# Yasas1994/Jaeger

Hardware: AMD Instinct MI355X
Metric: Mbp/s classified (1500bp frags) (higher is better)
Workload: dtype f16x3 (split-f16, f32 accumulate)

## Files before the change

jaeger_amd/csrc/jg_conv_f16_impl.h:

```cpp
#include <stdio.h>
#include <stdlib.h>
#include <type_traits>

#include "jg_common.h"

#include "jg_conv_dev.h"

namespace {


#ifdef JG_STAMP
static __device__ unsigned long long jg_stamp_acc[8];
#define JG_ST_DECL unsigned long long st_[8] = {0, 0, 0, 0, 0, 0, 0, 0}; unsigned long long st_t = __builtin_amdgcn_s_memtime(); const unsigned long long st_t0 = st_t
#define JG_ST(idx) do { const unsigned long long n_ = __builtin_amdgcn_s_memtime(); st_[idx] += n_ - st_t; st_t = n_; } while (0)
#define JG_ST_END do { st_[5] = __builtin_amdgcn_s_memtime() - st_t0; if (lane == 0) { for (int q_ = 0; q_ < 8; ++q_) atomicAdd(&jg_stamp_acc[q_], st_[q_]); } } while (0)
#else
#define JG_ST_DECL
#define JG_ST(idx)
#define JG_ST_END
#endif

#ifndef JG_PRIO
#define JG_PRIO 1
#endif
// ... 6 lines not shown
#ifndef JG_PAIRED
#define JG_PAIRED 1
#endif
#define JG_PRIO_MAIN() do { if (JG_PRIO) __builtin_amdgcn_s_setprio(2); } while (0)
#define JG_PRIO_EPI() do { if (JG_PRIO) __builtin_amdgcn_s_setprio(0); } while (0)

template <int K, unsigned EP, bool LUT = false, bool FLAT = false, int CW = 128, bool TANH = false, bool PIPE = false>
__global__ __launch_bounds__(LUT ? JG_LUT_WAVES * 64 : HT) __attribute__((amdgpu_waves_per_eu(K == 5 ? 2 : 1, 2)))
void conv_f16x3_kernel(ConvHArgs a) {
  constexpr int NTHR = LUT ? JG_LUT_WAVES * 64 : HT;
  constexpr int WA = K - 2;
  constexpr bool NARROW = !LUT && (CW == 64 || CW == 32);
  constexpr bool GEN = CW != 128;
  const int ch0 = GEN ? a.ch0 : 0;
  const int L_res = GEN ? a.L_res : a.L_out;
  constexpr int TM = NARROW ? 2 : 4;
  constexpr int TN = (NARROW && CW == 32) ? 1 : 2;
  constexpr int STRIPS = HM / (TM * 32);
  extern __shared__ __attribute__((aligned(16))) uint4 lds[];
  const int tid = threadIdx.x, lane = tid & 63;
  const int wid = __builtin_amdgcn_readfirstlane(tid >> 6);
  const int wm = LUT ? (wid & 1) : (NARROW ? wid : (wid >> 1));
  const int wn = LUT ? ((GEN && a.lut_one_half) ? 0 : (int)(blockIdx.x & 1u)) : (NARROW ? 0 : (wid & 1));
  const int i = lane & 31, h = lane >> 5;
  const int lut_sh = (LUT && !(GEN && a.lut_one_half)) ? 1 : 0;
  const int vgrid = (int)(gridDim.x >> lut_sh);
  int vb = (int)(blockIdx.x >> lut_sh);
  if ((vgrid & 7) == 0) vb = (vb & 7) * (vgrid >> 3) + (vb >> 3);
  constexpr int TPER = LUT ? JG_LUT_WAVES / 2 : NT;
  const int tsub = LUT ? (wid >> 1) : 0;
  const int rows_a = HM + (K - 1) * a.dil;
  const int a_items = NT * 4 * rows_a;
  uint4 *Abuf = lds;
  uint4 *Wbuf = lds + 2 * a_items;
  const int lut_rows = a.k * (a.lut_vocab + 1);
  float *epiL = LUT ? reinterpret_cast<float *>(lds) + lut_rows * LUT_RS
                    : reinterpret_cast<float *>(Wbuf + K * W_ITEMS);
  for (int q = tid; q < a.n_epi_rows * 2 * HN; q += NTHR) epiL[q] = a.epi[q];
  const unsigned lds0 = (unsigned)(size_t)(__attribute__((address_space(3))) void *)lds;
  const unsigned ldsA = __builtin_amdgcn_readfirstlane(lds0 + wid * 1024);
  const unsigned ldsW = __builtin_amdgcn_readfirstlane(lds0 + 2 * a_items * 16 + wid * 1024);

  const int n_tiles = FLAT ? a.flat_tiles : a.rows * a.tiles_m;
  const int n_pairs = (n_tiles + TPER - 1) / TPER;
  auto resolve = [&](const Tile &tile, int local, int len, int &row, int &p) -> bool {
    if constexpr (!FLAT) {
      row = tile.rowblk;
      p = tile.m0 + local;
      return tile.valid && p >= 0 && p < len;
    }
    const int v = tile.T * HM + local;
    if (v < 0 || !tile.valid) { row = 0; p = 0; return false; }
    int g, u, f;
    udivmod24(v, a.flat_wp, a.flat_inv_wp, g, u);
    udivmod24(u, a.flat_p, a.flat_inv_p, f, p);
    row = g * a.flat_frames + f;
    return f < a.flat_frames && p < len && row < a.rows;
  };
  int my_pairs = 0;
  if (vb < n_pairs) my_pairs = (n_pairs - 1 - vb) / vgrid + 1;
  if (my_pairs == 0) return;

  unsigned a_pk[A_ITERS];
#pragma unroll
  for (int it = 0; it < A_ITERS; ++it) {
    const int q = tid + it * HT;
    const int ph = q / rows_a;
    a_pk[it] = ((unsigned)(ph >> 2) << 20) | ((unsigned)(ph & 3) << 16) | (unsigned)(q - ph * rows_a);
  }
  unsigned w_voff[W_ITERS];
#pragma unroll
  for (int it = 0; it < W_ITERS; ++it) {
    const int q = tid + it * HT;
    w_voff[it] = (unsigned)((((q >> 8) * K * a.cc_in * 2 + ((q >> 7) & 1)) * HN + (q & (HN - 1))) * 16);
  }

  auto tiles_of = [&](int pass, Tile *t) {
#pragma unroll
    for (int u = 0; u < NT; ++u) {
      const int T = (vb + pass * vgrid) * TPER + tsub + u;
      const int Tc = min(T, n_tiles - 1);
      t[u].rowblk = Tc / a.tiles_m;
      t[u].m0 = (Tc - t[u].rowblk * a.tiles_m) * HM;
      t[u].valid = T < n_tiles;
      t[u].T = Tc;
    }
  };

  const uint8_t *bsrc = a.ids != nullptr ? a.ids : a.mask_in;
  unsigned char raw[A_ITERS];
  unsigned x_voff[A_ITERS];
  unsigned x_ok = 0;
  auto piece_pos = [&](const Tile *tl2, int it, int &pc, bool &inr) -> int {
    const int a_u = (int)(a_pk[it] >> 20), a_r = (int)(a_pk[it] & 0xffff);
    int rb, p;
    inr = resolve(tl2[0], a_r - a.pad_left, a.L_in, rb, p) && a_u < NT;
    pc = min(max(p, 0), a.L_in - 1);
    if constexpr (FLAT) rb = min(rb, a.rows - 1);
    return rb;
  };
  auto load_bytes = [&](const Tile *tl2) {
    if (bsrc != nullptr) {
#pragma unroll
      for (int it = 0; it < A_ITERS; ++it) {
        int pc; bool inr;
        const int rb = piece_pos(tl2, it, pc, inr);
        raw[it] = bsrc[(size_t)rb * a.L_in + pc];
      }
    } else {
#pragma unroll
      for (int it = 0; it < A_ITERS; ++it) raw[it] = 1;
    }
  };
  auto build_pieces = [&](const Tile *tl2) {
    x_ok = 0;
#pragma unroll
    for (int it = 0; it < A_ITERS; ++it) {
      int pc; bool inr;
      const int rb = piece_pos(tl2, it, pc, inr);
      const unsigned ph = (a_pk[it] >> 16) & 3;
      const unsigned byte = raw[it];
      bool keep;
      if (a.ids != nullptr) {
        x_voff[it] = (byte * a.cc_in * 4 + ph) * 16;
        keep = byte != 0 || !a.mask_from_ids;
      } else {
        x_voff[it] = (unsigned)(((rb * a.cc_row * 4 + (int)ph) * a.L_in + pc) * 16);
        keep = byte != 0;
      }
      if (inr && keep) x_ok |= 1u << it;
    }
  };
  const char *x_base = a.ids != nullptr ? reinterpret_cast<const char *>(a.embh)
                                        : reinterpret_cast<const char *>(a.xh);
  const unsigned x_cc_stride = a.ids != nullptr ? 4u * 16u : 4u * (unsigned)a.L_in * 16u;

  const bool x_last_wave = __builtin_amdgcn_readfirstlane((int)((A_ITERS - 1) * HT + wid * 64 < 4 * rows_a)) != 0;
  auto issue_w = [&](int cc, int t) {
    if (a.dbg & 16) return;
    const char *sb = reinterpret_cast<const char *>(a.wh) + ((size_t)(t * a.cc_in * 2 + cc * 2) * HN) * 16;
#pragma unroll
    for (int it = 0; it < W_ITERS; ++it) glds16(sb, w_voff[it], ldsW + t * (W_ITEMS * 16) + it * (HT * 16));
  };
  auto issue_x = [&](int cc, int buf) {
    if (a.dbg & 8) return;
    const char *sb = x_base + (size_t)cc * x_cc_stride;
    const unsigned dst = ldsA + buf * (a_items * 16);
#pragma unroll
    for (int it = 0; it < A_ITERS - 1; ++it) glds16_nt(sb, x_voff[it], dst + it * (HT * 16));
    if (x_last_wave) {
      if ((a_pk[A_ITERS - 1] >> 20) < NT) glds16_nt(sb, x_voff[A_ITERS - 1], dst + (A_ITERS - 1) * (HT * 16));
    }
  };
  auto zero_fill = [&](int buf) {
    uint4 *A = Abuf + buf * a_items;
#pragma unroll
    for (int it = 0; it < A_ITERS; ++it)
      if ((a_pk[it] >> 20) < NT && !((x_ok >> it) & 1u)) A[tid + it * HT] = make_uint4(0u, 0u, 0u, 0u);
  };

  f32x16 acc[TM][TN];
  auto zero_acc = [&]() {
#pragma unroll
    for (int tm = 0; tm < TM; ++tm)
#pragma unroll
      for (int tn = 0; tn < TN; ++tn)
#pragma unroll
        for (int r = 0; r < 16; ++r) acc[tm][tn][r] = 0.f;
  };
  zero_acc();

  const int w_frag = h * HN + wn * 64 + i;
  const int x_frag = h * rows_a + wm * (TM * 32) + i;

  Tile cur[NT], np[NT];
  JG_ST_DECL;
  tiles_of(0, cur);
  tiles_of(1, np);
  unsigned char *stage = reinterpret_cast<unsigned char *>(epiL + JG_EPI_ROWS * 2 * HN) + wid * 256;
  unsigned char nxt[4] = {0, 0, 0, 0};
  auto lut_fetch = [&](const Tile &tl) {
#pragma unroll
    for (int q4 = 0; q4 < 4; ++q4) {
      const int p = tl.m0 + wm * (TM * 32) - a.pad_left + lane + 64 * q4;
      const int pc = min(max(p, 0), a.L_in - 1);
      const unsigned char b = a.ids[(size_t)tl.rowblk * a.L_in + pc];
      nxt[q4] = (tl.valid && p >= 0 && p < a.L_in) ? b : (unsigned char)a.lut_vocab;
    }
  };
  if constexpr (LUT) {
    float4 *T4 = reinterpret_cast<float4 *>(lds);
    const float4 *src = reinterpret_cast<const float4 *>(a.lut) + (size_t)wn * lut_rows * 16;
    for (int q = tid; q < lut_rows * 16; q += NTHR) T4[(q >> 4) * (LUT_RS / 4) + (q & 15)] = src[q];
    lut_fetch(cur[0]);
    __syncthreads();
  } else {
    load_bytes(cur);
    build_pieces(cur);
    load_bytes(np);
    issue_x(0, 0);
#pragma unroll
    for (int t = 0; t < ((K == 5 && JG_PAIRED) ? 4 : WA); ++t) issue_w(0, t);
  }
  int xc = 0;
#ifdef JG_VALU_PROBE
  float probe[8];
#pragma unroll
  for (int q = 0; q < 8; ++q) probe[q] = (float)(lane + q);
#endif
  JG_PRIO_MAIN();
  for (int pass = 0; pass < my_pairs; ++pass) {
    if constexpr (LUT) {
#pragma unroll
      for (int q4 = 0; q4 < 4; ++q4) stage[lane + 64 * q4] = nxt[q4];
      lut_fetch(np[0]);
      __builtin_amdgcn_s_waitcnt(0xc07f);
      __builtin_amdgcn_wave_barrier();
      const float *Tl = reinterpret_cast<const float *>(lds) + 4 * h;
      for (int t = 0; t < a.k; ++t) {
#pragma unroll
        for (int tm = 0; tm < TM; ++tm) {
          const int rowi = stage[tm * 32 + i + t * a.dil];
          const float *r = Tl + (t * (a.lut_vocab + 1) + rowi) * LUT_RS;
#pragma unroll
          for (int tn = 0; tn < TN; ++tn)
#pragma unroll
            for (int g = 0; g < 4; ++g) {
              const float4 v = *reinterpret_cast<const float4 *>(r + tn * 32 + 8 * g);
              acc[tm][tn][4 * g + 0] += v.x; acc[tm][tn][4 * g + 1] += v.y;
              acc[tm][tn][4 * g + 2] += v.z; acc[tm][tn][4 * g + 3] += v.w;
            }
        }
      }
      __builtin_amdgcn_wave_barrier();
    }
    if constexpr (PIPE) {
      static_assert(K == 5 && !LUT && CW == 128, "the pipelined main loop is built for the 128-channel five-tap convs");
      constexpr int DIL = 3;
      struct XF { uint4 h[2], l[2]; };
      struct WF { uint4 h[2], l[2]; };
      XF xf[2];
      WF wf[2];
      const uint4 *Wb = Wbuf + w_frag;
      auto ldx = [&](XF &f, const uint4 *A, int t, int tp) {
#pragma unroll
        for (int tq = 0; tq < 2; ++tq) {
          f.h[tq] = A[(tp * 2 + tq) * 32 + t * DIL];
          f.l[tq] = A[2 * rows_a + (tp * 2 + tq) * 32 + t * DIL];
        }
      };
      auto ldw = [&](WF &f, int t) {
#pragma unroll
        for (int tn = 0; tn < 2; ++tn) {
          f.h[tn] = Wb[t * W_ITEMS + tn * 32];
          f.l[tn] = Wb[t * W_ITEMS + 2 * HN + tn * 32];
        }
      };
      auto mm = [&](auto zero_c, const WF &w, const XF &x, int tp, auto &&between) {
        constexpr bool ZERO = decltype(zero_c)::value;
#pragma unroll
        for (int tq = 0; tq < 2; ++tq)
#pragma unroll
          for (int tn = 0; tn < 2; ++tn) {
            f32x16 &c = acc[tp * 2 + tq][tn];
            const half8 wh = *reinterpret_cast<const half8 *>(&w.h[tn]), wl = *reinterpret_cast<const half8 *>(&w.l[tn]);
            const half8 xh = *reinterpret_cast<const half8 *>(&x.h[tq]), xl = *reinterpret_cast<const half8 *>(&x.l[tq]);
            if constexpr (ZERO) {
              const f32x16 z = {0.f, 0.f, 0.f, 0.f, 0.f, 0.f, 0.f, 0.f, 0.f, 0.f, 0.f, 0.f, 0.f, 0.f, 0.f, 0.f};
              c = __builtin_amdgcn_mfma_f32_32x32x16_f16(wh, xl, z, 0, 0, 0);
            } else {
              c = __builtin_amdgcn_mfma_f32_32x32x16_f16(wh, xl, c, 0, 0, 0);
            }
            c = __builtin_amdgcn_mfma_f32_32x32x16_f16(wl, xh, c, 0, 0, 0);
            c = __builtin_amdgcn_mfma_f32_32x32x16_f16(wh, xh, c, 0, 0, 0);
            between(tq * 2 + tn);
          }
      };
      const bool last_pass_ = pass == my_pairs - 1;
      wait_vm<2 * W_ITERS>();
      zero_fill(0);
      __syncthreads();
      ldw(wf[0], 0);
      ldx(xf[0], Abuf + x_frag, 0, 0);
      for (int cp = 0; cp < a.cc_in / 2; ++cp) {
#pragma unroll
        for (int half = 0; half < 2; ++half) {
          const int cc = 2 * cp + half;
          const bool last_chunk = cc == a.cc_in - 1;
          const bool tail = last_chunk && last_pass_;
          const int ncc = last_chunk ? 0 : cc + 1;
          const uint4 *A = Abuf + half * a_items + x_frag;
          const uint4 *An = Abuf + (half ^ 1) * a_items + x_frag;
#pragma unroll
          for (int g = 0; g < 10; ++g) {
            const int t = g >> 1, tp = g & 1;
            const bool step_end = g == 3 || g == 7 || g == 9;
            const bool pass_end = g == 9 && last_chunk;
            if (step_end && !pass_end) {
              if (g == 3) {
                if (tail) wait_vm<W_ITERS>();
                else if (x_last_wave) wait_vm<W_ITERS + A_ITERS>();
                else wait_vm<W_ITERS + A_ITERS - 1>();
              } else if (g == 7) {
                if (tail) wait_vm<0>();
                else if (x_last_wave) wait_vm<2 * W_ITERS + A_ITERS>();
                else wait_vm<2 * W_ITERS + A_ITERS - 1>();
              } else {
                wait_vm<2 * W_ITERS>();
                zero_fill(half ^ 1);
              }
              __syncthreads();
// ... 334 lines not shown
#pragma unroll
          for (int r = 0; r < 16; ++r) pool_acc[r] = -INFINITY;
        }
        if (!(a.dbg & 32)) {
#pragma unroll
          for (int j = 0; j < 2; ++j) {
            f32x2 v[4];
#pragma unroll
            for (int r = 0; r < 4; ++r) v[r] = f32x2{x[8 * j + 2 * r], x[8 * j + 2 * r + 1]};
            auto st_affine = [&](int row) {
              const float *pr = epiL + (row * 2) * HN + nb + 4 * h + 16 * j;
              const float4 sc0 = *reinterpret_cast<const float4 *>(pr), sc1 = *reinterpret_cast<const float4 *>(pr + 8);
              const float4 of0 = *reinterpret_cast<const float4 *>(pr + HN), of1 = *reinterpret_cast<const float4 *>(pr + HN + 8);
              v[0] = __builtin_elementwise_fma(v[0], f32x2{sc0.x, sc0.y}, f32x2{of0.x, of0.y});
              v[1] = __builtin_elementwise_fma(v[1], f32x2{sc0.z, sc0.w}, f32x2{of0.z, of0.w});
              v[2] = __builtin_elementwise_fma(v[2], f32x2{sc1.x, sc1.y}, f32x2{of1.x, of1.y});
              v[3] = __builtin_elementwise_fma(v[3], f32x2{sc1.z, sc1.w}, f32x2{of1.z, of1.w});
            };
            auto st_add = [&]() {
              const u32x4 qh = j == 0 ? q.sh0 : q.sh1, ql = j == 0 ? q.sl0 : q.sl1;
              unsigned hx = qh[0], hy = qh[1], hz = qh[2], hw_ = qh[3];
              unsigned lx = ql[0], ly = ql[1], lz = ql[2], lw_ = ql[3];
              swap32(hx, hz); swap32(hy, hw_);
              swap32(lx, lz); swap32(ly, lw_);
              v[0] += f32x2{mix_sum<0>(hx, lx), mix_sum<1>(hx, lx)};
              v[1] += f32x2{mix_sum<0>(hy, ly), mix_sum<1>(hy, ly)};
              v[2] += f32x2{mix_sum<0>(hz, lz), mix_sum<1>(hz, lz)};
              v[3] += f32x2{mix_sum<0>(hw_, lw_), mix_sum<1>(hw_, lw_)};
            };
            auto st_gelu = [&]() {
#pragma unroll
              for (int r = 0; r < 4; ++r) v[r] = fast_gelu2(v[r]);
            };
            auto st_nmd = [&]() {
              const f32x2 mk2 = {mk, mk};
#pragma unroll
              for (int r = 0; r < 4; ++r) nmd2[4 * j + r] = __builtin_elementwise_fma(v[r], mk2, nmd2[4 * j + r]);
            };
            st_affine(0);
            if constexpr (EP & JG_EP_NMD1) st_nmd();
            if constexpr (N1 == 1) st_affine(1);
            if constexpr (HAS_ADD) st_add();
            if constexpr (EP & JG_EP_ACT1) st_gelu();
            if constexpr (EP & JG_EP_NMD2) st_nmd();
            if constexpr (N2 == 1) st_affine(N1 ? 2 : 1);
            if constexpr (EP & JG_EP_ACT2) st_gelu();
            if (a.out_f16s) {
              unsigned hp[4], lp[4];
#pragma unroll
              for (int r = 0; r < 4; ++r) {
                typedef _Float16 half2_t __attribute__((ext_vector_type(2)));
                const half2_t hh = {(_Float16)v[r].x, (_Float16)v[r].y};
                hp[r] = *reinterpret_cast<const unsigned *>(&hh);
                const half2_t ll = {(_Float16)mix_rem<0>(v[r].x, hp[r]), (_Float16)mix_rem<1>(v[r].y, hp[r])};
                lp[r] = *reinterpret_cast<const unsigned *>(&ll);
              }
              vmax = fmaxf(fmaxf(vmax, fmaxf(fabsf(v[0].x), fabsf(v[0].y))), fmaxf(fabsf(v[1].x), fabsf(v[1].y)));
              vmax = fmaxf(fmaxf(vmax, fmaxf(fabsf(v[2].x), fabsf(v[2].y))), fmaxf(fabsf(v[3].x), fabsf(v[3].y)));
              vnan = vnan || __builtin_isunordered(v[0].x, v[0].y) || __builtin_isunordered(v[1].x, v[1].y) ||
                     __builtin_isunordered(v[2].x, v[2].y) || __builtin_isunordered(v[3].x, v[3].y);
              swap32(hp[0], hp[2]); swap32(hp[1], hp[3]);
              swap32(lp[0], lp[2]); swap32(lp[1], lp[3]);
              if (live && !(a.dbg & 64)) {
                uint4 *yh = reinterpret_cast<uint4 *>(a.y);
                const unsigned it4 = ob[tm] + (unsigned)(2 * tn + j) * L4;
                const u32x4 vhi = {hp[0], hp[1], hp[2], hp[3]}, vlo = {lp[0], lp[1], lp[2], lp[3]};
                st_stream(vhi, reinterpret_cast<u32x4 *>(yh + it4));
                st_stream(vlo, reinterpret_cast<u32x4 *>(yh + it4 + 2u * (unsigned)a.L_out));
              }
            } else if (a.pool_out != nullptr) {
#pragma unroll
              for (int r = 0; r < 4; ++r) {
                pool_acc[8 * j + 2 * r] = mk != 0.f ? fmaxf(pool_acc[8 * j + 2 * r], v[r].x) : pool_acc[8 * j + 2 * r];
                pool_acc[8 * j + 2 * r + 1] = mk != 0.f ? fmaxf(pool_acc[8 * j + 2 * r + 1], v[r].y) : pool_acc[8 * j + 2 * r + 1];
              }
            } else if (live && !(a.dbg & 64)) {
              float *yf = reinterpret_cast<float *>(a.y) + (size_t)om[tm] * a.cout + nb + 4 * h + 16 * j;
              *reinterpret_cast<float4 *>(yf) = make_float4(v[0].x, v[0].y, v[1].x, v[1].y);
              *reinterpret_cast<float4 *>(yf + 8) = make_float4(v[2].x, v[2].y, v[3].x, v[3].y);
            }
          }
        }
        if (b + 2 < 8) fetch(q, b + 2);
        if (tm == 3) {
          if constexpr (HAS_NMD) {
            float na[16];
#pragma unroll
            for (int r = 0; r < 8; ++r) { na[2 * r] = nmd2[r].x; na[2 * r + 1] = nmd2[r].y; }
            const float rv = lane_reduce(na, [](float x_, float y_) { return x_ + y_; });
            int ch;
            const size_t slot = reduced_slot(tn, ch);
            if (i < 16 && tile.valid) a.nmd_out[slot] = rv;
          }
          if (a.pool_out != nullptr) {
            const float rv = lane_reduce(pool_acc, [](float x_, float y_) { return fmaxf(x_, y_); });
            int ch;
            const size_t slot = reduced_slot(tn, ch);
            if (i < 16 && tile.valid) a.pool_out[slot] = rv;
          }
        }
      };
#pragma unroll
      for (int bp = 0; bp < 4; ++bp) {
        do_block(2 * bp, in0);
        do_block(2 * bp + 1, in1);
      }
      if ((!(vmax <= 65000.0f) || vnan) && a.overflow != nullptr && a.dbg == 0) atomicOr(a.overflow, 1);
      JG_PRIO_MAIN();
    } else {
      JG_PRIO_EPI();
      float vmax = 0.f;
      bool vnan = false;
      float nmd_acc[16];
      float nmd_acc2[16];
      struct Pre {
        uint2 sh[4], sl[4];
        unsigned char mkb;
      };
      auto swap32 = [](unsigned &lo_half_keeps, unsigned &hi_half_keeps) {
        const auto r = __builtin_amdgcn_permlane32_swap(lo_half_keeps, hi_half_keeps, false, false);
        lo_half_keeps = r[0];
        hi_half_keeps = r[1];
      };
      auto item4 = [&](int row, int mc, int nb, int j) -> unsigned {
        const int G = ((nb + ch0) >> 3) + 2 * j + h;
        return (unsigned)(((row * (a.cout_pad >> 4) + (G >> 1)) * 4 + (G & 1)) * a.L_out + mc);
      };
      const bool psplit = GEN && a.psplit != 0;
      const int L_st = psplit ? ((a.L_out + 1) >> 1) : a.L_out;
      auto item4_out = [&](int row, int mc, int nb, int j) -> unsigned {
        if constexpr (GEN) {
          if (psplit) {
            const int G = ((nb + ch0) >> 3) + 2 * j + h, CC = a.cout_pad >> 4;
            return (unsigned)(((row * 2 * CC + (mc & 1) * CC + (G >> 1)) * 4 + (G & 1)) * L_st + (mc >> 1));
          }
        }
        return item4(row, mc, nb, j);
      };
      auto out_pos = [&](const Tile &tile, int tm, int &row, int &mc) -> bool {
        int p;
        bool live = resolve(tile, (wm * TM + tm) * 32 + i, L_res, row, p);
        if constexpr (GEN) {
          if (a.ostride == 2) {
            live = live && !(p & 1);
            p >>= 1;
          }
        }
        mc = live ? p : 0;
        if constexpr (FLAT) {
          if (!live) row = min(max(row, 0), a.rows - 1);
        }
        return live;
      };
      auto prefetch = [&](Pre &p, const Tile &tile, int tm, int tn) {
        const int nb = (wn * 2 + tn) * 32;
        int orow, mc;
        out_pos(tile, tm, orow, mc);
        p.mkb = a.mask_out != nullptr ? a.mask_out[(size_t)orow * a.L_out + mc] : (unsigned char)1;
        if (a.addh != nullptr && !(a.dbg & 128)) {
#pragma unroll
          for (int j = 0; j < 2; ++j) {
            const unsigned it4 = item4(orow, mc, (!GEN || nb + ch0 + 16 * j < a.cout) ? nb : 0, j);
            typedef unsigned u32x4 __attribute__((ext_vector_type(4)));
            const u32x4 nh = ld_stream(reinterpret_cast<const u32x4 *>(a.addh + it4));
            const u32x4 nl = ld_stream(reinterpret_cast<const u32x4 *>(a.addh + it4 + 2u * (unsigned)a.L_out));
            uint4 vh = make_uint4(nh[0], nh[1], nh[2], nh[3]);
            uint4 vl = make_uint4(nl[0], nl[1], nl[2], nl[3]);
            swap32(vh.x, vh.z); swap32(vh.y, vh.w);
            swap32(vl.x, vl.z); swap32(vl.y, vl.w);
            p.sh[2 * j] = make_uint2(vh.x, vh.y);  p.sh[2 * j + 1] = make_uint2(vh.z, vh.w);
            p.sl[2 * j] = make_uint2(vl.x, vl.y);  p.sl[2 * j + 1] = make_uint2(vl.z, vl.w);
          }
        } else {
#pragma unroll
          for (int g = 0; g < 4; ++g) p.sh[g] = p.sl[g] = make_uint2(0u, 0u);
        }
      };
      auto epi_block = [&](f32x16 &x, const Tile &tile, int tm, int tn) {
        Pre p;
        prefetch(p, tile, tm, tn);
        const int nb = (wn * 2 + tn) * 32;
        int orow_, mc_;
        const bool live = out_pos(tile, tm, orow_, mc_);
        const float mk = p.mkb != 0 ? 1.f : 0.f;
        auto st_affine = [&](int row) {
          const float *pr = epiL + (row * 2) * HN + nb + 4 * h;
#pragma unroll
          for (int g = 0; g < 4; ++g) {
            const float4 sc = *reinterpret_cast<const float4 *>(pr + 8 * g);
            const float4 of = *reinterpret_cast<const float4 *>(pr + HN + 8 * g);
            x[4 * g + 0] = fmaf(x[4 * g + 0], sc.x, of.x);
            x[4 * g + 1] = fmaf(x[4 * g + 1], sc.y, of.y);
            x[4 * g + 2] = fmaf(x[4 * g + 2], sc.z, of.z);
            x[4 * g + 3] = fmaf(x[4 * g + 3], sc.w, of.w);
          }
        };
        auto st_dyt = [&](int row, float alpha, int use_mask) {
          const float *pr = epiL + (row * 2) * HN + nb + 4 * h;
          const float mm = use_mask ? mk : 1.0f;
#pragma unroll
          for (int g = 0; g < 4; ++g) {
            const float4 ga = *reinterpret_cast<const float4 *>(pr + 8 * g);
            const float4 be = *reinterpret_cast<const float4 *>(pr + HN + 8 * g);
            x[4 * g + 0] = (fast_tanh(alpha * x[4 * g + 0]) * ga.x + be.x) * mm;
            x[4 * g + 1] = (fast_tanh(alpha * x[4 * g + 1]) * ga.y + be.y) * mm;
            x[4 * g + 2] = (fast_tanh(alpha * x[4 * g + 2]) * ga.z + be.z) * mm;
            x[4 * g + 3] = (fast_tanh(alpha * x[4 * g + 3]) * ga.w + be.w) * mm;
          }
        };
        auto st_add = [&]() {
#pragma unroll
          for (int g = 0; g < 4; ++g) {
            x[4 * g + 0] += mix_sum<0>(p.sh[g].x, p.sl[g].x);
            x[4 * g + 1] += mix_sum<1>(p.sh[g].x, p.sl[g].x);
            x[4 * g + 2] += mix_sum<0>(p.sh[g].y, p.sl[g].y);
            x[4 * g + 3] += mix_sum<1>(p.sh[g].y, p.sl[g].y);
          }
        };
        auto st_gelu = [&]() {
          constexpr bool TANH_ONLY = TANH || EP == JG_EP_RUNTIME ||
                                     (EP != JG_EP_GENERIC && ((((EP >> 1) & 3) == 2) || (((EP >> 6) & 3) == 2)));
          if (TANH_ONLY || a.act_kind == JG_ACT_GELU_TANH) {
#pragma unroll
            for (int r = 0; r < 16; ++r) x[r] = fast_gelu(x[r]);
          } else if (a.act_kind == JG_ACT_GELU_ERF) {
#pragma unroll
            for (int r = 0; r < 16; ++r) x[r] = gelu_erf(x[r]);
          } else {
#pragma unroll
            for (int r = 0; r < 16; ++r) x[r] = fmaxf(x[r], 0.0f);
          }
        };
        auto st_nmd = [&](int which = 0) {
          const float mkl = live ? mk : 0.f;
          if constexpr (EP == JG_EP_RUNTIME) {
            if (which) {
#pragma unroll
              for (int r = 0; r < 16; ++r) nmd_acc2[r] = fmaf(x[r], mkl, nmd_acc2[r]);
              return;
            }
          }
#pragma unroll
          for (int r = 0; r < 16; ++r) nmd_acc[r] = fmaf(x[r], mkl, nmd_acc[r]);
        };
        if constexpr (EP == JG_EP_GENERIC) {
          for (int q = 0; q < ((a.dbg & 32) ? 0 : a.n_hst); ++q) {
            const HStageArg st = a.hst[q];
            switch (st.kind) {
              case JG_HST_AFFINE: st_affine(st.pad_); break;
              case JG_HST_DYT: st_dyt(st.pad_, st.f0, st.arg); break;
              case JG_HST_ADD: st_add(); break;
              case JG_HST_ACT:
#pragma unroll
                for (int r = 0; r < 16; ++r) x[r] = jg_act(x[r], st.arg);
                break;
              case JG_HST_NMD: st_nmd(); break;
              case JG_HST_MASKMUL:
#pragma unroll
                for (int r = 0; r < 16; ++r) x[r] *= mk;
                break;
              default: break;
            }
          }
        } else if constexpr (EP == JG_EP_RUNTIME) {
          const unsigned e_ = a.ep_rt;
          const int n1 = (int)((e_ >> 1) & 3u), n2 = (int)((e_ >> 6) & 3u);
          st_affine(0);
          if (e_ & JG_EP_NMD1) st_nmd(0);
          if (n1 == 1) st_affine(1);
          else if (n1 == 2) st_dyt(1, a.alpha1, a.dytmask1);
          if (e_ & JG_EP_ADD) st_add();
          if (e_ & JG_EP_ACT1) st_gelu();
          if (e_ & JG_EP_NMD2) st_nmd((e_ & JG_EP_NMD1) ? 1 : 0);
          if (n2 == 1) st_affine(n1 ? 2 : 1);
          else if (n2 == 2) st_dyt(n1 ? 2 : 1, a.alpha2, a.dytmask2);
          if (e_ & JG_EP_ACT2) st_gelu();
        } else if (!(a.dbg & 32)) {
          constexpr int N1 = (EP >> 1) & 3, N2 = (EP >> 6) & 3;
          st_affine(0);
          if constexpr (EP & JG_EP_NMD1) st_nmd();
          if constexpr (N1 == 1) st_affine(1);
          if constexpr (N1 == 2) st_dyt(1, a.alpha1, a.dytmask1);
          if constexpr (EP & JG_EP_ADD) st_add();
          if constexpr (EP & JG_EP_ACT1) st_gelu();
          if constexpr (EP & JG_EP_NMD2) st_nmd();
          if constexpr (N2 == 1) st_affine(N1 ? 2 : 1);
          if constexpr (N2 == 2) st_dyt(N1 ? 2 : 1, a.alpha2, a.dytmask2);
          if constexpr (EP & JG_EP_ACT2) st_gelu();
        }
        if constexpr (GEN) {
          if (psplit) {
#pragma unroll
            for (int r = 0; r < 16; ++r) x[r] *= mk;
          }
        }
        if (a.out_f16s) {
          uint2 ph[4], pl[4];
#pragma unroll
          for (int g = 0; g < 4; ++g) {
            half4 hh4, ll4;
#pragma unroll
            for (int j = 0; j < 4; ++j) {
              hh4[j] = (_Float16)x[4 * g + j];
              vmax = fmaxf(vmax, fabsf(x[4 * g + j]));
            }
            vnan = vnan || __builtin_isunordered(x[4 * g + 0], x[4 * g + 1]) || __builtin_isunordered(x[4 * g + 2], x[4 * g + 3]);
            ph[g] = *reinterpret_cast<uint2 *>(&hh4);
            ll4[0] = (_Float16)mix_rem<0>(x[4 * g + 0], ph[g].x);
            ll4[1] = (_Float16)mix_rem<1>(x[4 * g + 1], ph[g].x);
            ll4[2] = (_Float16)mix_rem<0>(x[4 * g + 2], ph[g].y);
            ll4[3] = (_Float16)mix_rem<1>(x[4 * g + 3], ph[g].y);
            pl[g] = *reinterpret_cast<uint2 *>(&ll4);
          }
#pragma unroll
          for (int j = 0; j < 2; ++j) {
            unsigned h0 = ph[2 * j].x, h1 = ph[2 * j].y, h2 = ph[2 * j + 1].x, h3 = ph[2 * j + 1].y;
            unsigned l0 = pl[2 * j].x, l1 = pl[2 * j].y, l2 = pl[2 * j + 1].x, l3 = pl[2 * j + 1].y;
            swap32(h0, h2); swap32(h1, h3);
            swap32(l0, l2); swap32(l1, l3);
            x[4 * j + 0] = __uint_as_float(h0); x[4 * j + 1] = __uint_as_float(h1);
            x[4 * j + 2] = __uint_as_float(h2); x[4 * j + 3] = __uint_as_float(h3);
            x[8 + 4 * j + 0] = __uint_as_float(l0); x[8 + 4 * j + 1] = __uint_as_float(l1);
            x[8 + 4 * j + 2] = __uint_as_float(l2); x[8 + 4 * j + 3] = __uint_as_float(l3);
          }
        }
      };
      auto store_block = [&](const f32x16 &x, const Tile &tile, int tm, int tn) {
        const int nb = (wn * 2 + tn) * 32;
        int orow, mc;
        const bool live = out_pos(tile, tm, orow, mc);
        if (live && !(a.dbg & 64)) {
          if (a.out_f16s) {
            uint4 *yh = reinterpret_cast<uint4 *>(a.y);
#pragma unroll
            for (int j = 0; j < 2; ++j) {
              if (GEN && nb + ch0 + 16 * j >= a.cout) continue;
              const unsigned it4 = item4_out(orow, mc, nb, j);
              typedef unsigned u32x4 __attribute__((ext_vector_type(4)));
              const u32x4 vhi = {__float_as_uint(x[4 * j]), __float_as_uint(x[4 * j + 1]),
                                 __float_as_uint(x[4 * j + 2]), __float_as_uint(x[4 * j + 3])};
              const u32x4 vlo = {__float_as_uint(x[8 + 4 * j]), __float_as_uint(x[8 + 4 * j + 1]),
                                 __float_as_uint(x[8 + 4 * j + 2]), __float_as_uint(x[8 + 4 * j + 3])};
              st_stream(vhi, reinterpret_cast<u32x4 *>(yh + it4));
              st_stream(vlo, reinterpret_cast<u32x4 *>(yh + it4 + 2u * (unsigned)L_st));
              if (GEN && psplit && (a.L_out & 1) && mc == a.L_out - 1) {
                const unsigned itz = it4 + (unsigned)((a.cout_pad >> 4) * 4 * L_st);
                const u32x4 z = {0u, 0u, 0u, 0u};
                st_stream(z, reinterpret_cast<u32x4 *>(yh + itz));
                st_stream(z, reinterpret_cast<u32x4 *>(yh + itz + 2u * (unsigned)L_st));
              }
            }
          } else {
            float *yf = reinterpret_cast<float *>(a.y) + ((size_t)orow * a.L_out + mc) * a.cout + ch0 + nb + 4 * h;
#pragma unroll
            for (int g = 0; g < 4; ++g)
              if (ch0 + nb + 8 * g + 4 * h < a.cout)
                *reinterpret_cast<float4 *>(yf + 8 * g) =
                    make_float4(x[4 * g], x[4 * g + 1], x[4 * g + 2], x[4 * g + 3]);
          }
        }
      };
#define JG_DPP(v, ctrl) __uint_as_float((unsigned)__builtin_amdgcn_update_dpp(0, (int)__float_as_uint(v), (ctrl), 0xf, 0xf, false))
      auto lane_reduce = [&](const float (&in)[16], auto op) -> float {
        const bool b2 = (i & 4) != 0, b1 = (i & 2) != 0, b0 = (i & 1) != 0, b3 = (i & 8) != 0;
        float s8[8], s4[4], s2[2];
#pragma unroll
        for (int q = 0; q < 8; ++q) {
          const float keep = b2 ? in[8 + q] : in[q], send = b2 ? in[q] : in[8 + q];
          s8[q] = op(keep, JG_DPP(send, 0x141));
        }
#pragma unroll
        for (int q = 0; q < 4; ++q) {
          const float keep = b1 ? s8[4 + q] : s8[q], send = b1 ? s8[q] : s8[4 + q];
          s4[q] = op(keep, JG_DPP(send, 0x4e));
        }
#pragma unroll
        for (int q = 0; q < 2; ++q) {
          const float keep = b0 ? s4[2 + q] : s4[q], send = b0 ? s4[q] : s4[2 + q];
          s2[q] = op(keep, JG_DPP(send, 0xb1));
        }
        const float keep1 = b3 ? s2[1] : s2[0], send1 = b3 ? s2[0] : s2[1];
        const float v = op(keep1, JG_DPP(send1, 0x128));
        return op(v, __shfl_xor(v, 16, 32));
      };
      auto reduced_slot = [&](const Tile &tile, int tn, int &ch) -> size_t {
        const int r = 8 * (int)((i & 4) != 0) + 4 * (int)((i & 2) != 0) + 2 * (int)((i & 1) != 0) + (int)((i & 8) != 0);
        ch = ch0 + (wn * 2 + tn) * 32 + 8 * (r >> 2) + 4 * h + (r & 3);
        return ((size_t)tile.T * STRIPS + wm) * a.cout + ch;
      };
      auto nmd_flush = [&](const Tile &tile, int tn) {
        const float v = lane_reduce(nmd_acc, [](float x, float y) { return x + y; });
        int ch;
        const size_t slot = reduced_slot(tile, tn, ch);
        if (i < 16 && tile.valid && ch < a.cout) a.nmd_out[slot] = v;
      };
      const bool has_nmd = (EP == JG_EP_GENERIC || EP == JG_EP_RUNTIME) ? a.nmd_out != nullptr : (EP & (JG_EP_NMD1 | JG_EP_NMD2)) != 0;
#pragma unroll
      for (int tn = 0; tn < TN; ++tn) {
#pragma unroll
        for (int r = 0; r < 16; ++r) nmd_acc[r] = 0.f;
        if constexpr (EP == JG_EP_RUNTIME) {
#pragma unroll
          for (int r = 0; r < 16; ++r) nmd_acc2[r] = 0.f;
        }
#pragma unroll
        for (int tm = 0; tm < TM; ++tm) epi_block(acc[tm][tn], cur[0], tm, tn);
        if (has_nmd) nmd_flush(cur[0], tn);
        if constexpr (EP == JG_EP_RUNTIME) {
          if (a.nmd_out2 != nullptr) {
            const float v2 = lane_reduce(nmd_acc2, [](float x, float y) { return x + y; });
            int ch2;
            const size_t slot2 = reduced_slot(cur[0], tn, ch2);
            if (i < 16 && cur[0].valid && ch2 < a.cout) a.nmd_out2[slot2] = v2;
          }
        }
      }
      if (a.pool_out != nullptr) {
        float mkv[TM];
#pragma unroll
        for (int tm = 0; tm < TM; ++tm) {
          int orow, mc;
          const bool live = out_pos(cur[0], tm, orow, mc);
          const unsigned char mb = a.mask_out != nullptr ? a.mask_out[(size_t)orow * a.L_out + mc] : (unsigned char)1;
          mkv[tm] = (live && mb != 0) ? 1.f : 0.f;
        }
#pragma unroll
        for (int tn = 0; tn < TN; ++tn) {
          float pa[16];
#pragma unroll
          for (int r = 0; r < 16; ++r) pa[r] = -INFINITY;
#pragma unroll
          for (int tm = 0; tm < TM; ++tm)
#pragma unroll
            for (int r = 0; r < 16; ++r) pa[r] = mkv[tm] != 0.f ? fmaxf(pa[r], acc[tm][tn][r]) : pa[r];
          const float v = lane_reduce(pa, [](float x, float y) { return fmaxf(x, y); });
          int ch;
          const size_t slot = reduced_slot(cur[0], tn, ch);
          if (i < 16 && cur[0].valid && ch < a.cout) a.pool_out[slot] = v;
        }
      } else {
#pragma unroll
        for (int tm = 0; tm < TM; ++tm) {
#pragma unroll
          for (int tn = 0; tn < TN; ++tn) store_block(acc[tm][tn], cur[0], tm, tn);
        }
      }
      if ((!(vmax <= 65000.0f) || vnan) && a.overflow != nullptr && a.dbg == 0) atomicOr(a.overflow, 1);
      JG_PRIO_MAIN();
    }
    if constexpr (!PIPE) zero_acc();
#pragma unroll
    for (int u = 0; u < NT; ++u) cur[u] = np[u];
    tiles_of(pass + 2, np);
    if constexpr (!LUT) load_bytes(np);
    JG_ST(4);
  }
#ifdef JG_VALU_PROBE
  if (probe[0] + probe[1] + probe[2] + probe[3] + probe[4] + probe[5] + probe[6] + probe[7] == 12345.678f) a.overflow[0] = 4;
#endif
  JG_ST_END;
}

template <int K, unsigned EP, bool FLAT = false, int CW = 128, bool TANH = false, bool PIPE = false>
int launch_ke(jg_engine *e, const ConvHArgs &a, hipStream_t s) {
  const int smem = jg_conv_f16_lds_bytes(K, a.dil);
  static bool attr_set = false;
  if (!attr_set) {
    JG_HIP(hipFuncSetAttribute(reinterpret_cast<const void *>(conv_f16x3_kernel<K, EP, false, FLAT, CW, TANH, PIPE>),
                               hipFuncAttributeMaxDynamicSharedMemorySize, 160 * 1024));
    attr_set = true;
  }
  const int n_tiles = FLAT ? a.flat_tiles : a.rows * a.tiles_m;
  const int n_pairs = (n_tiles + NT - 1) / NT;
  static const bool one_wg = jg_exp_env("JG_ONE_WG") != nullptr;
  int grid = ((smem <= 80 * 1024 && !one_wg) ? 2 : 1) * e->n_cu;
  if (grid > n_pairs) grid = n_pairs;
  ConvHArgs b = a;
  hipLaunchKernelGGL((conv_f16x3_kernel<K, EP, false, FLAT, CW, TANH, PIPE>), dim3((unsigned)grid), dim3(HT), (size_t)smem, s, b);
  JG_HIP(hipGetLastError());
#ifdef JG_STAMP
  {
    unsigned long long h[8], z[8] = {0, 0, 0, 0, 0, 0, 0, 0};
    JG_HIP(hipStreamSynchronize(s));
    JG_HIP(hipMemcpyFromSymbol(h, HIP_SYMBOL(jg_stamp_acc), sizeof(h)));
    JG_HIP(hipMemcpyToSymbol(HIP_SYMBOL(jg_stamp_acc), z, sizeof(z)));
    const double tot = (double)h[5];
    fprintf(stderr, "STAMP k=%d ep=%u rows=%d grid=%d total_cyc/wave=%.0f wait=%.3f barrier=%.3f issue=%.3f lds_mfma=%.3f epilogue=%.3f\n",
            K, EP, a.rows, grid, tot / (grid * 4.0), h[0] / tot, h[1] / tot, h[2] / tot, (h[3] + h[6]) / tot, h[4] / tot);
  }
#endif
  return JG_OK;
}

template <int K, unsigned EP, bool FLAT>
int launch_hot(jg_engine *e, const ConvHArgs &a, hipStream_t s) {
  if constexpr (K == 5) {
#ifdef JG_EXPERIMENT
    if (e->conv_pc == 2 && a.dil == 3 && a.cc_in % 2 == 0 && a.dbg == 0) return launch_ke<5, EP, FLAT, 128, true, true>(e, a, s);
#endif
    return launch_ke<5, EP, FLAT, 128, true>(e, a, s);
  } else {
    return launch_ke<K, EP, FLAT>(e, a, s);
  }
}

#if JG_CONV_PART == 4
template <unsigned EP, int CW, bool TANH = false>
int launch_lut_e(jg_engine *e, const ConvHArgs &a, hipStream_t s) {
  const int smem = jg_conv_lut_lds_bytes(a.k, a.lut_vocab);
  static bool attr_set = false;
  if (!attr_set) {
    JG_HIP(hipFuncSetAttribute(reinterpret_cast<const void *>(conv_f16x3_kernel<0, EP, true, false, CW, TANH>),
                               hipFuncAttributeMaxDynamicSharedMemorySize, 160 * 1024));
    attr_set = true;
  }
  const int n_tiles = a.rows * a.tiles_m;
  constexpr int tper = JG_LUT_WAVES / 2;
  const int n_pairs = (n_tiles + tper - 1) / tper;
  const int grid = a.lut_one_half ? (n_pairs < e->n_cu ? n_pairs : e->n_cu)
                                  : 2 * (n_pairs < e->n_cu / 2 ? n_pairs : e->n_cu / 2);
  hipLaunchKernelGGL((conv_f16x3_kernel<0, EP, true, false, CW, TANH>), dim3((unsigned)grid), dim3(JG_LUT_WAVES * 64), (size_t)smem, s, a);
  JG_HIP(hipGetLastError());
  return JG_OK;
}

int launch_lut(jg_engine *e, const ConvHArgs &a, hipStream_t s) {
  switch (a.ep) {
#define JG_CASE(ep) case (ep): return a.cout == 128 ? launch_lut_e<(ep), 128>(e, a, s) : launch_lut_e<(ep), 129>(e, a, s);
    JG_CASE(0u)
    JG_CASE(JG_EP_NMD1)
    JG_CASE(JG_EP_ACT1)
    JG_CASE(JG_EP_NORM1_AFF | JG_EP_ACT1)
    JG_CASE(JG_EP_NORM1_DYT | JG_EP_ACT1)
    case (JG_EP_NMD1 | JG_EP_NORM1_AFF | JG_EP_ACT1):
      if (a.cout == 128 && a.act_kind == JG_ACT_GELU_TANH) return launch_lut_e<(JG_EP_NMD1 | JG_EP_NORM1_AFF | JG_EP_ACT1), 128, true>(e, a, s);
      return a.cout == 128 ? launch_lut_e<(JG_EP_NMD1 | JG_EP_NORM1_AFF | JG_EP_ACT1), 128>(e, a, s)
                           : launch_lut_e<(JG_EP_NMD1 | JG_EP_NORM1_AFF | JG_EP_ACT1), 129>(e, a, s);
    JG_CASE(JG_EP_NMD1 | JG_EP_NORM1_DYT | JG_EP_ACT1)
    JG_CASE(JG_EP_ACT1 | JG_EP_NORM2_AFF)
    JG_CASE(JG_EP_RUNTIME)
#undef JG_CASE
    default: break;
  }
  jg_set_error("conv lut: stage pattern 0x%x has no compiled epilogue", a.ep);
  return JG_ERR_UNSUPPORTED;
}

#endif

#define JG_ROW_CASES(K)                                                                              \
  switch (a.ep) {                                                                                    \
    case 0u: return launch_ke<K, 0u>(e, a, s);                 \
    case (JG_EP_NMD1): return launch_ke<K, (JG_EP_NMD1)>(e, a, s);                                   \
    case (JG_EP_ACT1):                                    \
      if (K == 5 && a.act_kind == JG_ACT_GELU_TANH) return launch_hot<K, (JG_EP_ACT1), false>(e, a, s); \
      return launch_ke<K, (JG_EP_ACT1)>(e, a, s);                                                     \
    case (JG_EP_NORM1_AFF | JG_EP_ACT1): return launch_ke<K, (JG_EP_NORM1_AFF | JG_EP_ACT1)>(e, a, s); \
    case (JG_EP_NORM1_DYT | JG_EP_ACT1): return launch_ke<K, (JG_EP_NORM1_DYT | JG_EP_ACT1)>(e, a, s); \
    case (JG_EP_ADD | JG_EP_ACT1):                                                                   \
      if (K == 5 && a.act_kind == JG_ACT_GELU_TANH) return launch_hot<K, (JG_EP_ADD | JG_EP_ACT1), false>(e, a, s); \
      return launch_ke<K, (JG_EP_ADD | JG_EP_ACT1)>(e, a, s);                                         \
    case (JG_EP_NORM1_DYT | JG_EP_ADD | JG_EP_ACT1):                                                 \
      return launch_ke<K, (JG_EP_NORM1_DYT | JG_EP_ADD | JG_EP_ACT1)>(e, a, s);                      \
    case (JG_EP_ADD | JG_EP_ACT1 | JG_EP_NMD2 | JG_EP_NORM2_AFF | JG_EP_ACT2):                       \
      if (K == 5 && a.act_kind == JG_ACT_GELU_TANH)                                                  \
        return launch_hot<K, (JG_EP_ADD | JG_EP_ACT1 | JG_EP_NMD2 | JG_EP_NORM2_AFF | JG_EP_ACT2), false>(e, a, s); \
      return launch_ke<K, (JG_EP_ADD | JG_EP_ACT1 | JG_EP_NMD2 | JG_EP_NORM2_AFF | JG_EP_ACT2)>(e, a, s); \
    case (JG_EP_NORM1_DYT | JG_EP_ADD | JG_EP_ACT1 | JG_EP_NMD2 | JG_EP_NORM2_DYT | JG_EP_ACT2):     \
      return launch_ke<K, (JG_EP_NORM1_DYT | JG_EP_ADD | JG_EP_ACT1 | JG_EP_NMD2 | JG_EP_NORM2_DYT | JG_EP_ACT2)>(e, a, s); \
    case (JG_EP_NMD1 | JG_EP_NORM1_AFF | JG_EP_ACT1):                                                \
      return launch_ke<K, (JG_EP_NMD1 | JG_EP_NORM1_AFF | JG_EP_ACT1)>(e, a, s);                     \
    case (JG_EP_NMD1 | JG_EP_NORM1_DYT | JG_EP_ACT1):                                                \
      return launch_ke<K, (JG_EP_NMD1 | JG_EP_NORM1_DYT | JG_EP_ACT1)>(e, a, s);                     \
    case (JG_EP_ADD | JG_EP_ACT1 | JG_EP_NORM2_AFF | JG_EP_ACT2):                                    \
      return launch_ke<K, (JG_EP_ADD | JG_EP_ACT1 | JG_EP_NORM2_AFF | JG_EP_ACT2)>(e, a, s);         \
    case (JG_EP_NORM1_DYT | JG_EP_ADD | JG_EP_ACT1 | JG_EP_NORM2_DYT | JG_EP_ACT2):                  \
      return launch_ke<K, (JG_EP_NORM1_DYT | JG_EP_ADD | JG_EP_ACT1 | JG_EP_NORM2_DYT | JG_EP_ACT2)>(e, a, s); \
    case (JG_EP_ACT1 | JG_EP_NORM2_AFF): return launch_ke<K, (JG_EP_ACT1 | JG_EP_NORM2_AFF)>(e, a, s); \
    case (JG_EP_ACT1 | JG_EP_NORM2_AFF | JG_EP_ACT2):                                                \
      return launch_ke<K, (JG_EP_ACT1 | JG_EP_NORM2_AFF | JG_EP_ACT2)>(e, a, s);                     \
    case (JG_EP_NMD1 | JG_EP_NORM1_AFF | JG_EP_ADD | JG_EP_ACT1):                                    \
      return launch_ke<K, (JG_EP_NMD1 | JG_EP_NORM1_AFF | JG_EP_ADD | JG_EP_ACT1)>(e, a, s);         \
    case (JG_EP_NMD1 | JG_EP_NORM1_AFF | JG_EP_ADD | JG_EP_ACT1 | JG_EP_NORM2_AFF | JG_EP_ACT2):     \
      return launch_ke<K, (JG_EP_NMD1 | JG_EP_NORM1_AFF | JG_EP_ADD | JG_EP_ACT1 | JG_EP_NORM2_AFF | JG_EP_ACT2)>(e, a, s); \
    case (JG_EP_ADD | JG_EP_ACT1 | JG_EP_NMD2):            \
      return launch_ke<K, (JG_EP_ADD | JG_EP_ACT1 | JG_EP_NMD2)>(e, a, s);                           \
    case (JG_EP_NORM1_DYT | JG_EP_ADD | JG_EP_ACT1 | JG_EP_NMD2):                                    \
      return launch_ke<K, (JG_EP_NORM1_DYT | JG_EP_ADD | JG_EP_ACT1 | JG_EP_NMD2)>(e, a, s);         \
    case (JG_EP_NORM1_DYT): return launch_ke<K, (JG_EP_NORM1_DYT)>(e, a, s);                         \
    case (JG_EP_RUNTIME): return launch_ke<K, (JG_EP_RUNTIME)>(e, a, s);                             \
    default: break;                                                                                  \
  }                                                                                                  \
  jg_set_error("conv_f16x3: stage pattern 0x%x has no compiled epilogue", a.ep);                     \
  return JG_ERR_UNSUPPORTED;

}

#if JG_CONV_PART == 1
int jg_conv_f16_part_k5(jg_engine *e, const ConvHArgs &a, hipStream_t s) { JG_ROW_CASES(5) }
#elif JG_CONV_PART == 2
// ... 101 lines not shown
```

Baseline: 80.81.

## Precompute epilogue output offsets per tile and reload kernel args from kernarg segment

For non-generic epilogues, per-tm output and mask offsets plus liveness bits are computed once per tile. Prefetch, mask lookup and store then reuse these offsets instead of calling resolve/out_pos repeatedly. Kernel argument pointers are re-read from the kernarg segment behind opaque asm barriers, so the compiler does not keep them live in scalar registers across the main loop. The zero-fill predicate is also folded into a precomputed bitmask. The aim is to cut epilogue integer address work and register pressure, at the cost of more code paths and fragile 32-bit offset arithmetic.

After: 82.04, median of 6. +1.5%, better.

```diff
diff --git a/jaeger_amd/csrc/jg_conv_f16_impl.h b/jaeger_amd/csrc/jg_conv_f16_impl.h
--- a/jaeger_amd/csrc/jg_conv_f16_impl.h
+++ b/jaeger_amd/csrc/jg_conv_f16_impl.h
@@ -182,11 +182,15 @@
       if ((a_pk[A_ITERS - 1] >> 20) < NT) glds16_nt(sb, x_voff[A_ITERS - 1], dst + (A_ITERS - 1) * (HT * 16));
     }
   };
+  unsigned a_has = 0;
+#pragma unroll
+  for (int it = 0; it < A_ITERS; ++it) a_has |= ((a_pk[it] >> 20) < NT ? 1u : 0u) << it;
   auto zero_fill = [&](int buf) {
     uint4 *A = Abuf + buf * a_items;
+    const unsigned zf = a_has & ~x_ok;
 #pragma unroll
     for (int it = 0; it < A_ITERS; ++it)
-      if ((a_pk[it] >> 20) < NT && !((x_ok >> it) & 1u)) A[tid + it * HT] = make_uint4(0u, 0u, 0u, 0u);
+      if ((zf >> it) & 1u) A[tid + it * HT] = make_uint4(0u, 0u, 0u, 0u);
   };
 
   f32x16 acc[TM][TN];
@@ -827,18 +831,83 @@
         }
         return live;
       };
+      constexpr bool OPOS = !GEN;
+      unsigned ob[TM], om[TM], olive = 0;
+      size_t o_row = 0, o_mrow = 0;
+      unsigned o_step = 0;
+      const void *e_y = a.y, *e_addh = a.addh;
+      const uint8_t *e_mask = a.mask_out;
+      int e_dbg = a.dbg, e_f16s = a.out_f16s;
+      float *e_pool = a.pool_out, *e_nmd = a.nmd_out;
+      int *e_overflow = a.overflow;
+      if constexpr (OPOS) {
+        typedef const __attribute__((address_space(4))) ConvHArgs *KArgs;
+        KArgs ka = (KArgs)__builtin_amdgcn_kernarg_segment_ptr();
+        asm volatile("" : "+s"(ka));
+        e_addh = ka->addh;
+        e_mask = ka->mask_out;
+        e_dbg = ka->dbg;
+        e_f16s = ka->out_f16s;
+        e_nmd = ka->nmd_out;
+        const unsigned Lo = (unsigned)ka->L_out, CC4 = (unsigned)(ka->cout_pad >> 4) * 4u;
+        o_step = FLAT ? 2u * Lo : 32u * Lo;
+        asm volatile("" : "+s"(o_step));
+        if constexpr (!FLAT) {
+          o_row = (size_t)cur[0].rowblk * CC4 * Lo * 16u + (size_t)(wn * 8) * o_step;
+          o_mrow = (size_t)cur[0].rowblk * Lo;
+        }
+#pragma unroll
+        for (int tm = 0; tm < TM; ++tm) {
+          int row, p;
+          const bool live = resolve(cur[0], (wm * TM + tm) * 32 + i, (int)Lo, row, p);
+          const int mc = live ? p : 0;
+          if constexpr (FLAT) {
+            if (!live) row = min(max(row, 0), a.rows - 1);
+          }
+          if (live) olive |= 1u << tm;
+          if constexpr (FLAT) {
+            om[tm] = (unsigned)row * Lo + (unsigned)mc;
+            ob[tm] = ((unsigned)row * CC4 + (unsigned)h) * Lo + (unsigned)mc;
+          } else {
+            om[tm] = (unsigned)mc;
+            ob[tm] = ((unsigned)h * Lo + (unsigned)mc) * 16u;
+          }
+        }
+      }
+      auto o_item = [&](const void *base, int tm, int tn, int j, int plane) -> const char * {
+        if constexpr (FLAT) {
+          return reinterpret_cast<const char *>(base) + ((size_t)(ob[tm] + (unsigned)(((wn * 2 + tn) * 2 + j) * 2 + plane) * o_step) << 4);
+        } else {
+          return reinterpret_cast<const char *>(base) + (o_row + (size_t)((unsigned)((tn * 2 + j) * 2 + plane) * o_step)) + ob[tm];
+        }
+      };
+      auto o_maskbyte = [&](int tm) -> unsigned char {
+        return e_mask != nullptr ? (e_mask + o_mrow)[om[tm]] : (unsigned char)1;
+      };
       auto prefetch = [&](Pre &p, const Tile &tile, int tm, int tn) {
         const int nb = (wn * 2 + tn) * 32;
-        int orow, mc;
-        out_pos(tile, tm, orow, mc);
-        p.mkb = a.mask_out != nullptr ? a.mask_out[(size_t)orow * a.L_out + mc] : (unsigned char)1;
-        if (a.addh != nullptr && !(a.dbg & 128)) {
+        int orow = 0, mc = 0;
+        if constexpr (OPOS) {
+          p.mkb = o_maskbyte(tm);
+        } else {
+          out_pos(tile, tm, orow, mc);
+          p.mkb = a.mask_out != nullptr ? a.mask_out[(size_t)orow * a.L_out + mc] : (unsigned char)1;
+        }
+        if (e_addh != nullptr && !(e_dbg & 128)) {
 #pragma unroll
           for (int j = 0; j < 2; ++j) {
-            const unsigned it4 = item4(orow, mc, (!GEN || nb + ch0 + 16 * j < a.cout) ? nb : 0, j);
             typedef unsigned u32x4 __attribute__((ext_vector_type(4)));
-            const u32x4 nh = ld_stream(reinterpret_cast<const u32x4 *>(a.addh + it4));
-            const u32x4 nl = ld_stream(reinterpret_cast<const u32x4 *>(a.addh + it4 + 2u * (unsigned)a.L_out));
+            const u32x4 *src_h, *src_l;
+            if constexpr (OPOS) {
+              src_h = reinterpret_cast<const u32x4 *>(o_item(e_addh, tm, tn, j, 0));
+              src_l = reinterpret_cast<const u32x4 *>(o_item(e_addh, tm, tn, j, 1));
+            } else {
+              const unsigned it4 = item4(orow, mc, (!GEN || nb + ch0 + 16 * j < a.cout) ? nb : 0, j);
+              src_h = reinterpret_cast<const u32x4 *>(a.addh + it4);
+              src_l = reinterpret_cast<const u32x4 *>(a.addh + it4 + 2u * (unsigned)a.L_out);
+            }
+            const u32x4 nh = ld_stream(src_h);
+            const u32x4 nl = ld_stream(src_l);
             uint4 vh = make_uint4(nh[0], nh[1], nh[2], nh[3]);
             uint4 vl = make_uint4(nl[0], nl[1], nl[2], nl[3]);
             swap32(vh.x, vh.z); swap32(vh.y, vh.w);
@@ -855,8 +924,13 @@
         Pre p;
         prefetch(p, tile, tm, tn);
         const int nb = (wn * 2 + tn) * 32;
-        int orow_, mc_;
-        const bool live = out_pos(tile, tm, orow_, mc_);
+        bool live;
+        if constexpr (OPOS) {
+          live = ((olive >> tm) & 1u) != 0u;
+        } else {
+          int orow_, mc_;
+          live = out_pos(tile, tm, orow_, mc_);
+        }
         const float mk = p.mkb != 0 ? 1.f : 0.f;
         auto st_affine = [&](int row) {
           const float *pr = epiL + (row * 2) * HN + nb + 4 * h;
@@ -919,7 +993,7 @@
           for (int r = 0; r < 16; ++r) nmd_acc[r] = fmaf(x[r], mkl, nmd_acc[r]);
         };
         if constexpr (EP == JG_EP_GENERIC) {
-          for (int q = 0; q < ((a.dbg & 32) ? 0 : a.n_hst); ++q) {
+          for (int q = 0; q < ((e_dbg & 32) ? 0 : a.n_hst); ++q) {
             const HStageArg st = a.hst[q];
             switch (st.kind) {
               case JG_HST_AFFINE: st_affine(st.pad_); break;
@@ -950,7 +1024,7 @@
           if (n2 == 1) st_affine(n1 ? 2 : 1);
           else if (n2 == 2) st_dyt(n1 ? 2 : 1, a.alpha2, a.dytmask2);
           if (e_ & JG_EP_ACT2) st_gelu();
-        } else if (!(a.dbg & 32)) {
+        } else if (!(e_dbg & 32)) {
           constexpr int N1 = (EP >> 1) & 3, N2 = (EP >> 6) & 3;
           st_affine(0);
           if constexpr (EP & JG_EP_NMD1) st_nmd();
@@ -969,7 +1043,7 @@
             for (int r = 0; r < 16; ++r) x[r] *= mk;
           }
         }
-        if (a.out_f16s) {
+        if (e_f16s) {
           uint2 ph[4], pl[4];
 #pragma unroll
           for (int g = 0; g < 4; ++g) {
@@ -1000,12 +1074,35 @@
           }
         }
       };
-      auto store_block = [&](const f32x16 &x, const Tile &tile, int tm, int tn) {
+      char *f32_base = nullptr;
+      auto store_block = [&](const f32x16 &x, const Tile &tile, int tm, int tn, bool f16s) {
         const int nb = (wn * 2 + tn) * 32;
+        if constexpr (OPOS) {
+          typedef unsigned u32x4 __attribute__((ext_vector_type(4)));
+          if (f16s) {
+#pragma unroll
+            for (int j = 0; j < 2; ++j) {
+              const u32x4 vhi = {__float_as_uint(x[4 * j]), __float_as_uint(x[4 * j + 1]),
+                                 __float_as_uint(x[4 * j + 2]), __float_as_uint(x[4 * j + 3])};
+              const u32x4 vlo = {__float_as_uint(x[8 + 4 * j]), __float_as_uint(x[8 + 4 * j + 1]),
+                                 __float_as_uint(x[8 + 4 * j + 2]), __float_as_uint(x[8 + 4 * j + 3])};
+              st_stream(vhi, reinterpret_cast<u32x4 *>(const_cast<char *>(o_item(e_y, tm, tn, j, 0))));
+              st_stream(vlo, reinterpret_cast<u32x4 *>(const_cast<char *>(o_item(e_y, tm, tn, j, 1))));
+            }
+          } else {
+            char *yf = f32_base + tn * (32 * 4);
+            if constexpr (FLAT) yf += ((size_t)om[tm] * (HN * 4) + 16 * h);
+            else yf += om[tm] * (unsigned)(HN * 4) + 16u * (unsigned)h;
+#pragma unroll
+            for (int g = 0; g < 4; ++g)
+              *reinterpret_cast<float4 *>(yf + 32 * g) = make_float4(x[4 * g], x[4 * g + 1], x[4 * g + 2], x[4 * g + 3]);
+          }
+          return;
+        }
         int orow, mc;
         const bool live = out_pos(tile, tm, orow, mc);
-        if (live && !(a.dbg & 64)) {
-          if (a.out_f16s) {
+        if (live && !(e_dbg & 64)) {
+          if (e_f16s) {
             uint4 *yh = reinterpret_cast<uint4 *>(a.y);
 #pragma unroll
             for (int j = 0; j < 2; ++j) {
@@ -1067,9 +1164,9 @@
         const float v = lane_reduce(nmd_acc, [](float x, float y) { return x + y; });
         int ch;
         const size_t slot = reduced_slot(tile, tn, ch);
-        if (i < 16 && tile.valid && ch < a.cout) a.nmd_out[slot] = v;
-      };
-      const bool has_nmd = (EP == JG_EP_GENERIC || EP == JG_EP_RUNTIME) ? a.nmd_out != nullptr : (EP & (JG_EP_NMD1 | JG_EP_NMD2)) != 0;
+        if (i < 16 && tile.valid && ch < a.cout) e_nmd[slot] = v;
+      };
+      const bool has_nmd = (EP == JG_EP_GENERIC || EP == JG_EP_RUNTIME) ? e_nmd != nullptr : (EP & (JG_EP_NMD1 | JG_EP_NMD2)) != 0;
 #pragma unroll
       for (int tn = 0; tn < TN; ++tn) {
 #pragma unroll
@@ -1090,13 +1187,28 @@
           }
         }
       }
-      if (a.pool_out != nullptr) {
+      if constexpr (OPOS) {
+        typedef const __attribute__((address_space(4))) ConvHArgs *KArgs;
+        KArgs ka = (KArgs)__builtin_amdgcn_kernarg_segment_ptr();
+        asm volatile("" : "+s"(ka));
+        e_y = ka->y;
+        e_pool = ka->pool_out;
+        e_overflow = ka->overflow;
+      }
+      if (e_pool != nullptr) {
         float mkv[TM];
 #pragma unroll
         for (int tm = 0; tm < TM; ++tm) {
-          int orow, mc;
-          const bool live = out_pos(cur[0], tm, orow, mc);
-          const unsigned char mb = a.mask_out != nullptr ? a.mask_out[(size_t)orow * a.L_out + mc] : (unsigned char)1;
+          bool live;
+          unsigned char mb;
+          if constexpr (OPOS) {
+            live = ((olive >> tm) & 1u) != 0u;
+            mb = o_maskbyte(tm);
+          } else {
+            int orow, mc;
+            live = out_pos(cur[0], tm, orow, mc);
+            mb = a.mask_out != nullptr ? a.mask_out[(size_t)orow * a.L_out + mc] : (unsigned char)1;
+          }
           mkv[tm] = (live && mb != 0) ? 1.f : 0.f;
         }
 #pragma unroll
@@ -1111,16 +1223,33 @@
           const float v = lane_reduce(pa, [](float x, float y) { return fmaxf(x, y); });
           int ch;
           const size_t slot = reduced_slot(cur[0], tn, ch);
-          if (i < 16 && cur[0].valid && ch < a.cout) a.pool_out[slot] = v;
+          if (i < 16 && cur[0].valid && ch < a.cout) e_pool[slot] = v;
+        }
+      } else if constexpr (OPOS) {
+        auto store_tile = [&](bool f16s) {
+#pragma unroll
+          for (int tm = 0; tm < TM; ++tm) {
+            if (!((olive >> tm) & 1u)) continue;
+#pragma unroll
+            for (int tn = 0; tn < TN; ++tn) store_block(acc[tm][tn], cur[0], tm, tn, f16s);
+          }
+        };
+        if (!(e_dbg & 64)) {
+          if (e_f16s) {
+            store_tile(true);
+          } else {
+            f32_base = reinterpret_cast<char *>(const_cast<void *>(e_y)) + (o_mrow * (size_t)HN + (size_t)(wn * 64)) * 4u;
+            store_tile(false);
+          }
         }
       } else {
 #pragma unroll
         for (int tm = 0; tm < TM; ++tm) {
 #pragma unroll
-          for (int tn = 0; tn < TN; ++tn) store_block(acc[tm][tn], cur[0], tm, tn);
+          for (int tn = 0; tn < TN; ++tn) store_block(acc[tm][tn], cur[0], tm, tn, false);
         }
       }
-      if ((!(vmax <= 65000.0f) || vnan) && a.overflow != nullptr && a.dbg == 0) atomicOr(a.overflow, 1);
+      if ((!(vmax <= 65000.0f) || vnan) && e_overflow != nullptr && e_dbg == 0) atomicOr(e_overflow, 1);
       JG_PRIO_MAIN();
     }
     if constexpr (!PIPE) zero_acc();
```
